# spvkgn/vorbis-aotuv-lancer

Hardware: AMD Instinct MI355X
Metric: realtime-stream-equivalents/node (44.1kHz stereo q5) + MDCT HBM GB/s (higher is better)
Workload: dtype f32

## Files before the change

### vorbis_aotuv_lancer_amd/csrc/tone_kernels.hip

```cpp
#include <hip/hip_runtime.h>
#include <stdint.h>
#include <stdlib.h>
#include <mutex>
#include "batch.h"
#include "kernels.h"

#define NEGINF -9999.f
#define VMIN(x, y) ((x) > (y) ? (y) : (x))
#define VMAX(x, y) ((x) < (y) ? (y) : (x))
#define TM_CHUNKS 16

namespace {

__device__ __forceinline__ int seed_key(float f)
{
    int v = __float_as_int(f);
    return v ^ ((v >> 31) & 0x7fffffff);
}
__device__ __forceinline__ float seed_val(int k) { return __int_as_float(k ^ ((k >> 31) & 0x7fffffff)); }

__device__ __forceinline__ unsigned chase_pop(unsigned m, const unsigned long long H, const unsigned ge)
{
    for (;;) {
        const unsigned m2 = m & (m - 1);
        if (!m2) break;
        const int k0 = __ffs((int)m) - 1, k1 = __ffs((int)m2) - 1;
        const unsigned c1 = (ge >> k0) & 1u;
        const unsigned c2 = (unsigned)(H >> (8 * k0 + (k1 - k0 - 1))) & 1u;
        if (!(c1 & c2)) break;
        m = m2;
    }
    return m;
}

__device__ __forceinline__ void chase_run(const unsigned short *__restrict__ gl, int i, unsigned m, const int own, const int oend,
                                          const bool last, unsigned long long &alive, unsigned &left7, unsigned &m_own,
                                          unsigned &m_next)
{
    unsigned long long H = 0;
#pragma unroll
    for (int b = 0; b < 7; b++) {
        const int q = i - 1 - b;
        if (q >= 0) H |= (unsigned long long)(gl[q] >> 8) << (8 * b);
    }
    for (; i < own; i += 4) {
        const unsigned long long g4 = *(const unsigned long long *)(gl + i);
#pragma unroll
        for (int u = 0; u < 4; u++) {
            const unsigned g = (unsigned)(g4 >> (16 * u)) & 0xffffu;
            m = chase_pop(m, H, g & 0xffu);
            m = ((m << 1) | 1u) & 0x7fu;
            H = (H << 8) | (g >> 8);
        }
    }
    m_own = m;
    unsigned long long F = 0;
    for (; i + 3 <= oend; i += 4) {
        const unsigned long long g4 = *(const unsigned long long *)(gl + i);
        unsigned nb = 0;
#pragma unroll
        for (int u = 0; u < 4; u++) {
            const unsigned g = (unsigned)(g4 >> (16 * u)) & 0xffffu;
            m = chase_pop(m, H, g & 0xffu);
            nb |= ((m >> 6) & 1u) << u;
            m = ((m << 1) | 1u) & 0x7fu;
            H = (H << 8) | (g >> 8);
        }
        F |= (unsigned long long)nb << (i - own);
    }
    if (i <= oend) {
        const unsigned long long g4 = *(const unsigned long long *)(gl + i);
        unsigned nb = 0;
#pragma unroll
        for (int u = 0; u < 3; u++) {
            if (i + u <= oend) {
                const unsigned g = (unsigned)(g4 >> (16 * u)) & 0xffffu;
                m = chase_pop(m, H, g & 0xffu);
                nb |= ((m >> 6) & 1u) << u;
                m = ((m << 1) | 1u) & 0x7fu;
                H = (H << 8) | (g >> 8);
            }
        }
        F |= (unsigned long long)nb << (i - own);
    }
    m_next = m;
    alive = F >> 7;
    left7 = (unsigned)F & 0x7fu;
    if (last) {
#pragma unroll
        for (int b = 0; b < 7; b++) {
            const int q = oend - b - own;
            const unsigned bit = (m >> b) & 1u;
            if (q >= 0) alive |= (unsigned long long)bit << q;
            else left7 |= bit << (q + 7);
        }
    }
}

template <int TM_NB>
__global__ __launch_bounds__(TM_NB * 32) void k_tonemask(vbm_batch b, const int runin)
{
    constexpr int TM_THREADS = TM_NB * 32;
    extern __shared__ __align__(16) int tm_lds[];
    __shared__ float s_att[TM_NB], s_dboff[TM_NB];
    __shared__ unsigned long long s_alive[TM_NB][TM_CHUNKS];
    const vbm_psy *p = &b.setup->psy[b.block_mode];
    const int n = p->n, tn = p->total_octave_lines, linesper = p->eighth_octave_lines;
    const int tnp = tn | 1;
    const int glp = (tn + 8) & ~7;
    float *seedF = (float *)tm_lds;
    unsigned short *glS = (unsigned short *)(tm_lds + TM_NB * tnp + (TM_NB & 1));
    const int tid = threadIdx.x;
    const int cb0 = blockIdx.x * TM_NB;
    if (cb0 >= vbm_ncb(b)) return;
    const int nblk = (vbm_ncb(b) - cb0 < TM_NB) ? vbm_ncb(b) - cb0 : TM_NB;

    for (int k = tid; k < TM_NB * tnp; k += TM_THREADS) seedF[k] = NEGINF;
    if (tid < TM_NB) {
        const int cb = cb0 + (tid < nblk ? tid : 0);
        float att = b.local_ampmax[cb] + p->ath_adjatt;
        if (att < p->ath_maxatt) att = p->ath_maxatt;
        s_att[tid] = att;
        s_dboff[tid] = p->max_curve_dB - b.global_ampmax[cb / b.ch];
    }
    __syncthreads();

    {
        const int ngroups = p->ngroups;
        const int4 *__restrict__ group_tab = (const int4 *)p->group_tab;
        const float *__restrict__ tonecurves = p->tonecurves;
        const int shiftoc = p->shiftoc, firstoc = p->firstoc;
        int blk = 0, g = tid;
        while (g >= ngroups) { g -= ngroups; blk++; }
        for (int item = tid; item < nblk * ngroups; item += TM_THREADS, g += TM_THREADS) {
            while (g >= ngroups) { g -= ngroups; blk++; }
            const float *f = b.logfft_bm + (size_t)(cb0 + blk) * n;
            const int4 rec = group_tab[g];
            const int s0 = rec.x, s1 = rec.y;
            float max = f[s0];
            for (int i = s0 + 1; i < s1; i += 4) {
                float v[4];
#pragma unroll
                for (int u = 0; u < 4; u++) v[u] = f[(i + u < s1) ? i + u : s1 - 1];
#pragma unroll
                for (int u = 0; u < 4; u++)
                    if (v[u] > max) max = v[u];
            }
            if (max + 6.f > __int_as_float(rec.z) + s_att[blk]) {
                long oc = rec.w;
                oc = oc >> shiftoc;
                if (oc >= VBM_P_BANDS) oc = VBM_P_BANDS - 1;
                if (oc < 0) oc = 0;
                const float *curves = tonecurves + (size_t)oc * VBM_P_LEVELS * (VBM_EHMER_MAX + 2);
                const int ocl = rec.w - firstoc;
                int choice = (int)(((double)(max + s_dboff[blk]) - 30.) * (double).1f);
                choice = VMAX(choice, 0);
                choice = VMIN(choice, VBM_P_LEVELS - 1);
                const float *posts = curves + choice * (VBM_EHMER_MAX + 2);
                const float *curve = posts + 2;
                const int post1 = (int)posts[1];
                int seedptr = (int)((float)ocl + (posts[0] - VBM_EHMER_OFFSET) * linesper - (linesper >> 1));
                float *row = seedF + blk * tnp;
                for (int i = (int)posts[0]; i < post1 && seedptr < tn; i += 8) {
                    float cv[8];
#pragma unroll
                    for (int u = 0; u < 8; u++) cv[u] = curve[(i + u < post1) ? i + u : post1 - 1];
#pragma unroll
                    for (int u = 0; u < 8; u++) {
                        if (i + u < post1 && seedptr < tn) {
                            if (seedptr > 0) (void)__hip_atomic_fetch_max(&row[seedptr], max + cv[u], __ATOMIC_RELAXED, __HIP_MEMORY_SCOPE_WORKGROUP);
                            seedptr += linesper;
                        }
                    }
                }
            }
        }
    }
    __syncthreads();

    {
        const int ngrp = (tn + 7) >> 3;
        int cblk = 0, cg = tid;
        for (int item = tid; item < nblk * ngrp; item += TM_THREADS, cg += TM_THREADS) {
            while (cg >= ngrp) { cg -= ngrp; cblk++; }
            const int j0 = cg << 3;
            const float *sd = seedF + cblk * tnp;
            float w[15];
#pragma unroll
            for (int t = 0; t < 15; t++) {
                int q = j0 - 7 + t;
                q = q < 0 ? 0 : (q < tn ? q : tn - 1);
                w[t] = sd[q];
            }
            unsigned r[4] = {0u, 0u, 0u, 0u};
#pragma unroll
            for (int u = 0; u < 8; u++) {
                const int j = j0 + u;
                unsigned ge = 0, le = 0;
#pragma unroll
                for (int k = 1; k <= 7; k++) {
                    if (j - k >= 0) {
                        if (!(w[7 + u] < w[7 + u - k])) ge |= 1u << (k - 1);
                        if (k <= 6 && w[7 + u] <= w[7 + u - k]) le |= 1u << (k - 1);
                    }
                }
                r[u >> 1] |= (ge | (le << 8)) << (16 * (u & 1));
            }
            *reinterpret_cast<uint4 *>(glS + cblk * glp + j0) = make_uint4(r[0], r[1], r[2], r[3]);
        }
    }
    __syncthreads();

    {
        const int blk = tid / TM_CHUNKS, c = tid % TM_CHUNKS;
        const int own = c * 64;
        const bool active = blk < nblk && own < tn;
        const unsigned short *gl = glS + blk * glp;
        unsigned long long alive = 0;
        unsigned m_own = 0, m_next = 0, used = 0, left7 = 0;
        const int oend = own + 63 < tn - 1 ? own + 63 : tn - 1;
        const bool last = own + 64 >= tn;
        if (active) {
            const int i0 = own >= runin ? own - runin : 0;
            chase_run(gl, i0, 0u, own, oend, last, alive, left7, m_own, m_next);
            used = m_own;
        }
        for (;;) {
            const unsigned truth = __shfl_up(m_next, 1);
            const bool redo = active && c > 0 && truth != used;
            if (!__any(redo)) break;
            if (redo) {
                chase_run(gl, own, truth, own, oend, last, alive, left7, m_own, m_next);
                used = truth;
            }
        }
        {
            const unsigned from_right = __shfl_down(left7, 1);
            if (active && !last) alive |= (unsigned long long)from_right << 57;
        }
        if (blk < nblk) s_alive[blk][c] = active ? alive : 0ull;
    }
    __syncthreads();

    {
        const int wave = tid >> 6, lane = tid & 63;
        for (int blk = wave; blk < nblk; blk += TM_THREADS / 64) {
            float *sd = seedF + blk * tnp;
            float am[TM_CHUNKS];
            int st[TM_CHUNKS], en[TM_CHUNKS];
            int carry = 0;
#pragma unroll
            for (int c = 0; c < TM_CHUNKS; c++) {
                am[c] = 0.f; st[c] = 0; en[c] = 0;
                if (c * 64 < tn) {
                    const unsigned long long w = s_alive[blk][c];
                    const int q = c * 64 + lane;
                    int endpos = 0;
                    if ((w >> lane) & 1ull) {
                        am[c] = sd[q];
                        const unsigned long long above = lane < 63 ? (w >> (lane + 1)) : 0ull;
                        int nq = -1;
                        if (above) nq = q + 1 + (__ffsll((long long)above) - 1);
                        else if (c + 1 < TM_CHUNKS && (c + 1) * 64 < tn) {
                            const unsigned long long w2 = s_alive[blk][c + 1];
                            if (w2) nq = (c + 1) * 64 + (__ffsll((long long)w2) - 1);
                        }
                        if (nq >= 0 && sd[nq] > am[c]) endpos = nq;
                        else endpos = q + linesper + 1;
                        if (endpos > tn) endpos = tn;
                    }
                    int incl = endpos;
                    { const int t = __builtin_amdgcn_update_dpp(0, incl, 0x111, 0xf, 0xf, true); incl = t > incl ? t : incl; }
                    { const int t = __builtin_amdgcn_update_dpp(0, incl, 0x112, 0xf, 0xf, true); incl = t > incl ? t : incl; }
                    { const int t = __builtin_amdgcn_update_dpp(0, incl, 0x114, 0xf, 0xf, true); incl = t > incl ? t : incl; }
                    { const int t = __builtin_amdgcn_update_dpp(0, incl, 0x118, 0xf, 0xf, true); incl = t > incl ? t : incl; }
                    { const int t = __builtin_amdgcn_update_dpp(0, incl, 0x142, 0xa, 0xf, false); incl = t > incl ? t : incl; }
                    { const int t = __builtin_amdgcn_update_dpp(0, incl, 0x143, 0xc, 0xf, false); incl = t > incl ? t : incl; }
                    int excl = __builtin_amdgcn_update_dpp(0, incl, 0x138, 0xf, 0xf, true);
                    if (carry > excl) excl = carry;
                    st[c] = excl;
                    en[c] = endpos;
                    const int tot = __builtin_amdgcn_readlane(incl, 63);
                    if (tot > carry) carry = tot;
                }
            }
#pragma unroll
            for (int c = 0; c < TM_CHUNKS; c++)
                if (c * 64 < tn)
                    for (int x = st[c]; x < en[c]; x++) sd[x] = am[c];
        }
    }
    __syncthreads();

    {
        const int blk = tid % TM_NB, r0 = tid / TM_NB;
        if (blk < nblk) {
            const int cb = cb0 + blk;
            float *out = b.toneT + (size_t)(cb >> 6) * b.slab_words + (cb & 63);
            const float *sd = seedF + blk * tnp;
            const float att = s_att[blk], tone_abs_limit = p->tone_abs_limit;
            const int *__restrict__ seg_p0 = p->seg_p0, *__restrict__ seg_p1 = p->seg_p1;
            const float *__restrict__ ath = p->ath;
            constexpr int STEP = TM_THREADS / TM_NB;
            for (int i0 = r0; i0 < n; i0 += 4 * STEP) {
                int q0[4], q1[4];
                float at[4];
#pragma unroll
                for (int u = 0; u < 4; u++) {
                    const int i = (i0 + u * STEP < n) ? i0 + u * STEP : r0;
                    q0[u] = seg_p0[i]; q1[u] = seg_p1[i]; at[u] = ath[i];
                }
#pragma unroll
                for (int u = 0; u < 4; u++) {
                    const int i = i0 + u * STEP;
                    if (i < n) {
                        float minV;
                        if (q0[u] < 0) {
                            minV = sd[tn - 1];
                        } else {
                            minV = sd[q0[u]];
                            if (minV > tone_abs_limit) minV = tone_abs_limit;
                            for (int pos = q0[u] + 1; pos <= q1[u]; pos++) {
                                const float sv = sd[pos];
                                if ((sv > NEGINF && sv < minV) || minV == NEGINF) minV = sv;
                            }
                        }
                        float v = at[u] + att;
                        if (v < minV) v = minV;
                        out[(size_t)i * 64] = v;
                    }
                }
            }
        }
    }
}

template <int NB>
int launch(const vbm_batch *b, int tn, size_t lds, hipStream_t st)
{
    const int runin = 16;
    {
        static std::mutex mu;
        static size_t allowed = 0;
        std::lock_guard<std::mutex> guard(mu);
        if (lds > allowed) {
            if (hipFuncSetAttribute(reinterpret_cast<const void *>(k_tonemask<NB>), hipFuncAttributeMaxDynamicSharedMemorySize,
                                    (int)lds) != hipSuccess) return -2;
            allowed = lds;
        }
    }
    hipLaunchKernelGGL(k_tonemask<NB>, dim3((unsigned)((b->ncb + NB - 1) / NB)), dim3(NB * 32), lds, st, *b, runin);
    return hipGetLastError() == hipSuccess ? 0 : -2;
}

size_t lds_bytes(int nb, int tn) { return (size_t)(nb * (tn | 1)) * 4 + (size_t)nb * ((tn + 8) & ~7) * 2 + 64; }

}

extern "C" int vbm_launch_tonemask(const vbm_batch *b, int tn, hipStream_t st)
{
    if (tn > TM_CHUNKS * 64 || tn < 2) return -2;
    return launch<8>(b, tn, lds_bytes(8, tn), st);
}
```

Baseline: 101,400.

## Replace iterative chase_pop loop with branchless bitmask step tracking le-state

Rewrites the tone-mask stack-chase so each step is a constant-time bitmask update. It carries a small 7-bit L state of le comparisons instead of a 56-bit history word H and a data-dependent pop loop. The chunk handoff state now packs m and L together, so speculative chunks only rerun when both match. This removes divergent while-loops and 64-bit shifts from the serial scan, at the cost of extra state in the carry comparison and a possible change in how often chunks must redo.

```diff
diff --git a/vorbis_aotuv_lancer_amd/csrc/tone_chase.h b/vorbis_aotuv_lancer_amd/csrc/tone_chase.h
--- /dev/null
+++ b/vorbis_aotuv_lancer_amd/csrc/tone_chase.h
@@ -0,0 +1,75 @@
+#pragma once
+
+#ifdef __HIPCC__
+#define TONE_CHASE_FN __host__ __device__ __forceinline__
+#else
+#define TONE_CHASE_FN static inline
+#endif
+
+TONE_CHASE_FN unsigned tone_chase_msb7(const unsigned m) { return 0x40000000u >> __builtin_clz((m << 1) | 1u); }
+
+TONE_CHASE_FN unsigned tone_chase_step(unsigned &m, unsigned &L, const unsigned ge, const unsigned le)
+{
+    const unsigned P = ge & L;
+    const unsigned t = m & ~P;
+    const unsigned mp = (m & (t | (0u - t))) | tone_chase_msb7(m);
+    const unsigned k0 = (unsigned)__builtin_ctz(mp | 0x40u);
+    const unsigned l = (le >> k0) & 1u;
+    L = ((L & mp) << 1) | l;
+    m = ((mp << 1) | 1u) & 0x7fu;
+    return mp;
+}
+
+TONE_CHASE_FN void chase_run(const unsigned short *__restrict__ gl, int i, unsigned m, unsigned L, const int own, const int oend,
+                             const bool last, unsigned long long &alive, unsigned &left7, unsigned &m_own, unsigned &L_own,
+                             unsigned &m_next, unsigned &L_next)
+{
+    for (; i < own; i += 4) {
+        const unsigned long long g4 = *(const unsigned long long *)(gl + i);
+#pragma unroll
+        for (int u = 0; u < 4; u++) {
+            const unsigned g = (unsigned)(g4 >> (16 * u)) & 0xffffu;
+            (void)tone_chase_step(m, L, g & 0xffu, g >> 8);
+        }
+    }
+    m_own = m;
+    L_own = L & 0x7fu;
+    unsigned long long F = 0;
+    for (; i + 3 <= oend; i += 4) {
+        const unsigned long long g4 = *(const unsigned long long *)(gl + i);
+        unsigned nb = 0;
+#pragma unroll
+        for (int u = 0; u < 4; u++) {
+            const unsigned g = (unsigned)(g4 >> (16 * u)) & 0xffffu;
+            const unsigned mp = tone_chase_step(m, L, g & 0xffu, g >> 8);
+            nb |= ((mp >> 6) & 1u) << u;
+        }
+        F |= (unsigned long long)nb << (i - own);
+    }
+    if (i <= oend) {
+        const unsigned long long g4 = *(const unsigned long long *)(gl + i);
+        unsigned nb = 0;
+#pragma unroll
+        for (int u = 0; u < 3; u++) {
+            if (i + u <= oend) {
+                const unsigned g = (unsigned)(g4 >> (16 * u)) & 0xffffu;
+                const unsigned mp = tone_chase_step(m, L, g & 0xffu, g >> 8);
+                nb |= ((mp >> 6) & 1u) << u;
+            }
+        }
+        F |= (unsigned long long)nb << (i - own);
+    }
+    m_next = m;
+    L_next = L & 0x7fu;
+    alive = F >> 7;
+    left7 = (unsigned)F & 0x7fu;
+    if (last) {
+#pragma unroll
+        for (int b = 0; b < 7; b++) {
+            const int q = oend - b - own;
+            const unsigned bit = (m >> b) & 1u;
+            if (q >= 0) alive |= (unsigned long long)bit << q;
+            else left7 |= bit << (q + 7);
+        }
+    }
+}
diff --git a/vorbis_aotuv_lancer_amd/csrc/tone_kernels.hip b/vorbis_aotuv_lancer_amd/csrc/tone_kernels.hip
--- a/vorbis_aotuv_lancer_amd/csrc/tone_kernels.hip
+++ b/vorbis_aotuv_lancer_amd/csrc/tone_kernels.hip
@@ -4,6 +4,7 @@
 #include <mutex>
 #include "batch.h"
 #include "kernels.h"
+#include "tone_chase.h"
 
 #define NEGINF -9999.f
 #define VMIN(x, y) ((x) > (y) ? (y) : (x))
@@ -18,84 +19,6 @@
     return v ^ ((v >> 31) & 0x7fffffff);
 }
 __device__ __forceinline__ float seed_val(int k) { return __int_as_float(k ^ ((k >> 31) & 0x7fffffff)); }
-
-__device__ __forceinline__ unsigned chase_pop(unsigned m, const unsigned long long H, const unsigned ge)
-{
-    for (;;) {
-        const unsigned m2 = m & (m - 1);
-        if (!m2) break;
-        const int k0 = __ffs((int)m) - 1, k1 = __ffs((int)m2) - 1;
-        const unsigned c1 = (ge >> k0) & 1u;
-        const unsigned c2 = (unsigned)(H >> (8 * k0 + (k1 - k0 - 1))) & 1u;
-        if (!(c1 & c2)) break;
-        m = m2;
-    }
-    return m;
-}
-
-__device__ __forceinline__ void chase_run(const unsigned short *__restrict__ gl, int i, unsigned m, const int own, const int oend,
-                                          const bool last, unsigned long long &alive, unsigned &left7, unsigned &m_own,
-                                          unsigned &m_next)
-{
-    unsigned long long H = 0;
-#pragma unroll
-    for (int b = 0; b < 7; b++) {
-        const int q = i - 1 - b;
-        if (q >= 0) H |= (unsigned long long)(gl[q] >> 8) << (8 * b);
-    }
-    for (; i < own; i += 4) {
-        const unsigned long long g4 = *(const unsigned long long *)(gl + i);
-#pragma unroll
-        for (int u = 0; u < 4; u++) {
-            const unsigned g = (unsigned)(g4 >> (16 * u)) & 0xffffu;
-            m = chase_pop(m, H, g & 0xffu);
-            m = ((m << 1) | 1u) & 0x7fu;
-            H = (H << 8) | (g >> 8);
-        }
-    }
-    m_own = m;
-    unsigned long long F = 0;
-    for (; i + 3 <= oend; i += 4) {
-        const unsigned long long g4 = *(const unsigned long long *)(gl + i);
-        unsigned nb = 0;
-#pragma unroll
-        for (int u = 0; u < 4; u++) {
-            const unsigned g = (unsigned)(g4 >> (16 * u)) & 0xffffu;
-            m = chase_pop(m, H, g & 0xffu);
-            nb |= ((m >> 6) & 1u) << u;
-            m = ((m << 1) | 1u) & 0x7fu;
-            H = (H << 8) | (g >> 8);
-        }
-        F |= (unsigned long long)nb << (i - own);
-    }
-    if (i <= oend) {
-        const unsigned long long g4 = *(const unsigned long long *)(gl + i);
-        unsigned nb = 0;
-#pragma unroll
-        for (int u = 0; u < 3; u++) {
-            if (i + u <= oend) {
-                const unsigned g = (unsigned)(g4 >> (16 * u)) & 0xffffu;
-                m = chase_pop(m, H, g & 0xffu);
-                nb |= ((m >> 6) & 1u) << u;
-                m = ((m << 1) | 1u) & 0x7fu;
-                H = (H << 8) | (g >> 8);
-            }
-        }
-        F |= (unsigned long long)nb << (i - own);
-    }
-    m_next = m;
-    alive = F >> 7;
-    left7 = (unsigned)F & 0x7fu;
-    if (last) {
-#pragma unroll
-        for (int b = 0; b < 7; b++) {
-            const int q = oend - b - own;
-            const unsigned bit = (m >> b) & 1u;
-            if (q >= 0) alive |= (unsigned long long)bit << q;
-            else left7 |= bit << (q + 7);
-        }
-    }
-}
 
 template <int TM_NB>
 __global__ __launch_bounds__(TM_NB * 32) void k_tonemask(vbm_batch b, const int runin)
@@ -217,20 +140,20 @@
         const bool active = blk < nblk && own < tn;
         const unsigned short *gl = glS + blk * glp;
         unsigned long long alive = 0;
-        unsigned m_own = 0, m_next = 0, used = 0, left7 = 0;
+        unsigned m_own = 0, L_own = 0, m_next = 0, L_next = 0, used = 0, left7 = 0;
         const int oend = own + 63 < tn - 1 ? own + 63 : tn - 1;
         const bool last = own + 64 >= tn;
         if (active) {
             const int i0 = own >= runin ? own - runin : 0;
-            chase_run(gl, i0, 0u, own, oend, last, alive, left7, m_own, m_next);
-            used = m_own;
+            chase_run(gl, i0, 0u, 0u, own, oend, last, alive, left7, m_own, L_own, m_next, L_next);
+            used = m_own | ((L_own & m_own) << 8);
         }
         for (;;) {
-            const unsigned truth = __shfl_up(m_next, 1);
+            const unsigned truth = __shfl_up(m_next | ((L_next & m_next) << 8), 1);
             const bool redo = active && c > 0 && truth != used;
             if (!__any(redo)) break;
             if (redo) {
-                chase_run(gl, own, truth, own, oend, last, alive, left7, m_own, m_next);
+                chase_run(gl, own, truth & 0x7fu, truth >> 8, own, oend, last, alive, left7, m_own, L_own, m_next, L_next);
                 used = truth;
             }
         }
```

After: 103,100 (median of 6 runs). 1.7% higher.
